# ku222/Attention-GAN

Hardware: AMD Instinct MI355X
Metric: train images/sec at 256×256 stage-3, batch 24/GPU, 1/2/4/8 MI355X (higher is better)
Workload: dtype f32; 1 GPU; full 3-stage AttnGAN 64->128->256 train step: G + 3xD updates + word attention + DAMSM words/sentence loss + KL + 4x fused Adam (BASELINE.json configs[2]); workload_key=full3, batch_per_gpu=24, global_batch=24, gf_dim=32, df_dim=64, emb_dim=256, seq_len=10, text_encoder=bypassed (frozen; N(0,1) embeddings), parallelism=dp1, discriminator_streams=3, launch=eager, gradient_exchange=none (one rank), losses_finite=True

## Files before the change

### attention-gan_amd/csrc/conv.hip

```cpp
#include "conv_common.h"

#include <cxxabi.h>
#include <cstdlib>


using namespace agan;

using namespace agan::conv;

namespace {

__global__ __launch_bounds__(256) void ktable_kernel(int2* __restrict__ tab, int n, int K, int RS, int S, int IHW, int IW, int DY) {
    const int k = blockIdx.x * 256 + threadIdx.x;
    if (k >= n) return;
    int2 a, b;
    if (k < K) {
        const int c = k / RS, rs = k - c * RS, r = rs / S, q = rs - r * S;
        const int dy = r * DY, dx = q * DY;
        a.x = c * IHW + dy * IW + dx;
        a.y = (dy & 0xFFFF) | (dx << 16);
        b.x = c * IHW * 4;
        b.y = rs * kTapRowBytes;
    } else {
        a.x = 0;
// ... 723 lines not shown
                int rl, rh;
                up_fwd_taps(py, r, rl, rh);
                if (a < rl || a > rh) continue;
                for (int px = 0; px < 2; ++px)
                    for (int q = 0; q < 2; ++q) {
                        int sl, sh;
                        up_fwd_taps(px, q, sl, sh);
                        if (b < sl || b > sh) continue;
                        v += dwk[((size_t)(py * 2 + px) * cout + co) * K + (ci * 4 + r * 2 + q)];
                    }
            }
        dw[e] = accumulate ? dw[e] + v : v;
    }
}

__global__ __launch_bounds__(256) void bias_grad_kernel(const float* __restrict__ dy, float* __restrict__ db, int B, int C,
                                                        int HW, int accumulate) {
    __shared__ float red[4];
    const int c = blockIdx.x;
    float s = 0.f;
    for (int b = 0; b < B; ++b) {
        const float* p = dy + ((size_t)b * C + c) * HW;
        for (int i = threadIdx.x; i < HW; i += 256) s += p[i];
    }
    s = block_sum<256>(s, red);
    if (threadIdx.x == 0) db[c] = accumulate ? db[c] + s : s;
}

}

static thread_local hipEvent_t g_timer_start = nullptr, g_timer_stop = nullptr;
static thread_local const void* g_timed_kernel = nullptr;
static thread_local int g_timed_split = 0;
namespace agan { namespace conv { thread_local const void* g_noted_kernel = nullptr; } }
static inline void timer_begin(hipStream_t st) {
    if (g_timer_start) (void)hipEventRecord(g_timer_start, st);
}
static inline void timer_end(hipStream_t st, int split) {
    if (g_timer_stop) {
        (void)hipEventRecord(g_timer_stop, st);
        g_timed_kernel = agan::conv::g_noted_kernel;
        g_timed_split = split;
    }
    g_timer_start = g_timer_stop = nullptr;
}
namespace agan { namespace conv {
void timed_begin(hipStream_t st) { timer_begin(st); }
void timed_end(hipStream_t st, int split) { timer_end(st, split); }
} }

static bool dt16(int dt) { return dt == AGAN_DT_BF16 || dt == AGAN_DT_F16; }
static int mode_dtype(int mode) { return mode == AGAN_PREC_BF16 ? AGAN_DT_BF16 : (mode == AGAN_PREC_F16 ? AGAN_DT_F16 : AGAN_DT_F32); }

enum class GatherPath { none, p16, patch, winograd, small_n, direct };
struct GatherRoute {
    int mode = AGAN_PREC_F32;
    GatherPath path = GatherPath::none;
    P16Plan p16{};
    PatchPlan pp{};
    PatchGather patch{};
    WinoPlan wino{};
    GatherPlan direct{};
    size_t ws_bytes = 0;
    int split = 1;
};

static GatherRoute route_gather(const agan_conv_geom* gg, int prec, int in_dtype, int out_dtype, bool epilogue) {
    GatherRoute r;
    auto take = [&r](GatherPath path, size_t ws_bytes, int split) {
        r.path = path;
        r.ws_bytes = ws_bytes;
        r.split = split;
        return r;
    };
    if (check_geom(gg)) return r;
    const Geom g = make_geom(gg);
    if (prec_planes(prec) > 0 && patch_supported(g)) r.mode = prec;
    const bool f32io = in_dtype == AGAN_DT_F32 && out_dtype == AGAN_DT_F32;
    if (const int want = mode_dtype(r.mode)) {
        if ((in_dtype == AGAN_DT_F32 || in_dtype == want) && (out_dtype == AGAN_DT_F32 || out_dtype == want)) {
            r.p16 = plan_p16(g, in_dtype != AGAN_DT_F32);
            if (r.p16.ok) return take(GatherPath::p16, r.p16.ws_bytes, r.p16.ksplit);
        }
    }
    if (r.mode != AGAN_PREC_F32) {
        if (!f32io) return r;
        r.pp = make_patch_plan(g);
        r.patch = plan_patch_gather(g, r.pp);
        return take(GatherPath::patch, r.patch.ws_bytes, r.patch.ksplit);
    }
    if (f32io && !epilogue) {
        r.wino = plan_wino(g);
        if (r.wino.ok) return take(GatherPath::winograd, r.wino.ws_bytes, r.wino.ksplit);
    }
    if (small_n_gather_supported(g)) {
        const bool linear = g.RS == 1 && g.IH == 1 && g.IW == 1;
        if ((in_dtype == AGAN_DT_F32 || (dt16(in_dtype) && !linear)) && out_dtype == AGAN_DT_F32) return take(GatherPath::small_n, 0, 1);
        return r;
    }
    if (in_dtype == AGAN_DT_F32 && (out_dtype == AGAN_DT_F32 || dt16(out_dtype))) {
        r.direct = plan_gather(g, AGAN_PREC_F32);
        return take(GatherPath::direct, r.direct.ws_bytes, r.direct.ksplit);
    }
    return r;
}

enum class WgradPath { none, winograd, rows, patch, small_n, direct };
struct WgradRoute {
    int mode = AGAN_PREC_F32;
    WgradPath path = WgradPath::none;
    WinoWgradPlan wino{};
    RowsPlan rows{};
    PatchPlan pp{};
    PatchWgrad patch{};
    SmallWgradPlan small{};
    WgradPlan direct{};
    size_t ws_bytes = 0;
    int split = 1;
};

static WgradRoute route_wgrad(const agan_conv_geom* gg, int pack_mode, int prec, int x_dtype, int dy_dtype) {
    WgradRoute r;
    auto take = [&r](WgradPath path, size_t ws_bytes, int split) {
        r.path = path;
        r.ws_bytes = ws_bytes;
        r.split = split;
        return r;
    };
    if (check_geom(gg)) return r;
    const Geom g = make_geom(gg);
    const bool up = pack_mode == AGAN_PACK_UP_FWD, x16 = x_dtype != AGAN_DT_F32, y16 = dy_dtype != AGAN_DT_F32;
    if (prec_planes(prec) > 0 && patch_supported(g)) {
        r.mode = prec;
        if (prec == AGAN_PREC_BF16X6) r.mode = AGAN_PREC_F16X3;
        if (up && !plan_rows_wgrad(g, r.mode, false, false, true).ok) r.mode = AGAN_PREC_F32;
    }
    if (x16 || y16) {
        const int want = mode_dtype(r.mode);
        const bool ok = r.mode == AGAN_PREC_F32
                            ? pack_mode == AGAN_PACK_FWD && small_n_wgrad_supported(g) && dt16(x_dtype) && !y16
                            : want != AGAN_DT_F32 && (!x16 || x_dtype == want) && (!y16 || dy_dtype == want);
        if (!ok) return r;
    }
    if (r.mode == AGAN_PREC_F32 && !up && !x16 && !y16) {
        r.wino = plan_wino_wgrad(g);
        if (r.wino.ok) return take(WgradPath::winograd, r.wino.ws_bytes, r.wino.psplit);
    }
    if (!(r.mode == AGAN_PREC_F32 && small_n_wgrad_supported(g))) {
        r.rows = plan_rows_wgrad(g, r.mode, x16, y16, up);
        if (r.rows.ok) return take(WgradPath::rows, r.rows.ws_bytes, r.rows.psplit);
    }
    if (r.mode != AGAN_PREC_F32) {
        r.pp = make_patch_plan(g);
        r.patch = plan_patch_wgrad(g, r.pp, r.mode);
        return take(WgradPath::patch, r.patch.ws_bytes, r.patch.psplit);
    }
    if (!up && small_n_wgrad_supported(g)) {
        r.small = plan_wgrad_small_n(g);
        return take(WgradPath::small_n, r.small.ws_bytes, r.small.nchunk);
    }
    if (!x16 && !y16) {
        r.direct = plan_wgrad(g, up);
        return take(WgradPath::direct, r.direct.ws_bytes, r.direct.psplit);
    }
    return r;
}

static int check_ws(const char* who, size_t need, const void* ws, size_t ws_bytes) {
    if (need > ws_bytes || (need && !ws)) {
        set_error("%s: workspace %zu < %zu", who, ws_bytes, need);
        return AGAN_EWORKSPACE;
    }
    return AGAN_OK;
}

template <class Launch>
static int launch_main(hipStream_t st, int split, const char* what, Launch&& launch) {
    timer_begin(st);
    launch();
    timer_end(st, split);
    return check_launch(what);
}

extern "C" {

int agan_timer_last_kernel(char* name, size_t capacity) {
    AGAN_REQUIRE(name && capacity > 1, "timer_last_kernel: bad argument");
    name[0] = 0;
    if (!g_timed_kernel) return AGAN_OK;
    const char* mangled = hipKernelNameRefByPtr(g_timed_kernel, nullptr);
    if (!mangled) return AGAN_OK;
    int status = 0;
    char* dem = abi::__cxa_demangle(mangled, nullptr, nullptr, &status);
    const char* src = (status == 0 && dem) ? dem : mangled;
    strncpy(name, src, capacity - 1);
    name[capacity - 1] = 0;
    free(dem);
    return AGAN_OK;
}

int agan_timer_last_split(void) { return g_timed_kernel ? g_timed_split : 0; }

int agan_timer_create(void** event) {
    AGAN_REQUIRE(event != nullptr, "timer_create: null pointer");
    hipEvent_t e;
    if (hipEventCreate(&e) != hipSuccess) {
        set_error("timer_create: hipEventCreate failed");
        return AGAN_ELAUNCH;
    }
    *event = e;
    return AGAN_OK;
}
int agan_timer_destroy(void* event) { return (event && hipEventDestroy(static_cast<hipEvent_t>(event)) != hipSuccess) ? AGAN_ELAUNCH : AGAN_OK; }
// ... 114 lines not shown
    return route_gather(gg, prec, in_dtype, out_dtype, false).path != GatherPath::none ? 1 : 0;
}

int agan_conv_gather_dt(const void* in_v, const void* wkv, const float* bias, void* out_v, const agan_conv_geom* gg, const int32_t* ktable,
                        int prec, int act, const void* lrelu_mask_v, void* ws, size_t ws_bytes, void* stream, const float* in_scale,
                        float* out_amax, int in_dtype, int out_dtype) {
    if (int e = check_geom(gg)) return e;
    AGAN_REQUIRE(in_v && wkv && out_v && ktable, "conv_gather: null pointer");
    AGAN_REQUIRE(act == AGAN_ACT_NONE || (act == AGAN_ACT_LRELU && gg->Cout > 4),
                 "conv_gather: fused activation %d not available for this call (MFMA paths, LeakyReLU only)", act);
    AGAN_REQUIRE(!lrelu_mask_v || (gg->Cout > 4 && act == AGAN_ACT_NONE),
                 "conv_gather: the LeakyReLU-derivative mask needs an MFMA path and no other activation");
    AGAN_REQUIRE(prec == AGAN_PREC_F32 || prec_planes(prec) > 0, "conv_gather: unknown precision mode %d", prec);
    const GatherRoute r = route_gather(gg, prec, in_dtype, out_dtype, bias || act != AGAN_ACT_NONE || lrelu_mask_v);
    AGAN_REQUIRE(r.mode == prec,
                 "conv_gather: precision mode %d does not take this geometry (agan_conv_effective_prec says which one does)", prec);
    AGAN_REQUIRE(r.path != GatherPath::none,
                 "conv_gather: 16-bit activation storage (%d -> %d) is not available for this geometry / precision %d "
                 "(agan_conv_gather_dt_supported)", in_dtype, out_dtype, prec);
    AGAN_REQUIRE(prec != AGAN_PREC_F16X3 || in_scale != nullptr, "conv_gather: AGAN_PREC_F16X3 needs the operand's agan_absmax_scale pair");
    if (int e = check_ws("conv_gather", r.ws_bytes, ws, ws_bytes)) return e;
    const Geom g = make_geom(gg);
    hipStream_t st = as_stream(stream);
    const float* in = static_cast<const float*>(in_v);
    const float* wk = static_cast<const float*>(wkv);
    const float* lrelu_mask = static_cast<const float*>(lrelu_mask_v);
    void* dst = r.split > 1 ? ws : out_v;
    const float* slabs = static_cast<const float*>(ws);
    size_t slab = 0;
    float* sum_amax = nullptr;
    int e = AGAN_OK;
    switch (r.path) {
        case GatherPath::p16:
            slab = r.p16.slab;
            e = launch_main(st, r.split, "conv_gather/p16", [&] {
                launch_p16_gather(in_v, wkv, bias, dst, g, r.p16, prec, act, lrelu_mask_v, st, in_dtype != AGAN_DT_F32, out_dtype != AGAN_DT_F32);
            });
            break;
        case GatherPath::patch:
            slab = r.patch.slab;
            sum_amax = out_amax;
            e = launch_main(st, r.split, "conv_gather/patch", [&] {
                launch_patch_gather(in, wkv, bias, static_cast<float*>(dst), g, r.pp, r.patch, prec, act, lrelu_mask, st, in_scale, out_amax);
            });
            break;
        case GatherPath::winograd:
            slab = r.wino.slab;
            slabs = reinterpret_cast<const float*>(static_cast<const char*>(ws) + r.wino.u_bytes);
            e = launch_main(st, r.split, "conv_gather/winograd", [&] { launch_wino(in, wk, static_cast<float*>(out_v), g, r.wino, ws, st); });
            break;
        case GatherPath::small_n:
            e = launch_main(st, r.split, "conv_gather/small_n", [&] { launch_gather_small_n(in_v, wk, bias, static_cast<float*>(out_v), g, st, in_dtype); });
            break;
        default: {
            const GatherPlan& p = r.direct;
            slab = p.slab;
            const int2* ktab = reinterpret_cast<const int2*>(ktable);
            e = launch_main(st, r.split, "conv_gather", [&] {
                if (p.bn == 128) launch_gather<128, 2, 2>(in, wk, bias, dst, ktab, g, p, act, lrelu_mask_v, st, out_dtype);
                else if (p.bn == 64) launch_gather<64, 2, 2>(in, wk, bias, dst, ktab, g, p, act, lrelu_mask_v, st, out_dtype);
                else launch_gather<32, 4, 1>(in, wk, bias, dst, ktab, g, p, act, lrelu_mask_v, st, out_dtype);
            });
        }
    }
    if (e || r.split == 1) return e;
    launch_sum_slabs(slabs, r.split, (size_t)g.B * g.Cout * g.OH * g.OW, slab, bias, g.Cout, g.OH * g.OW, out_v, 0, act, lrelu_mask_v, sum_amax, st,
                     out_dtype);
    return check_launch("conv_gather/sum_slabs");
}

int agan_conv_gather(const float* in, const void* wkv, const float* bias, float* out, const agan_conv_geom* gg, const int32_t* ktable,
                     int prec, int act, const float* lrelu_mask, void* ws, size_t ws_bytes, void* stream, const float* in_scale,
                     float* out_amax) {
    return agan_conv_gather_dt(in, wkv, bias, out, gg, ktable, prec, act, lrelu_mask, ws, ws_bytes, stream, in_scale, out_amax,
                               AGAN_DT_F32, AGAN_DT_F32);
}

static const int kPrecs[] = {AGAN_PREC_F32, AGAN_PREC_BF16, AGAN_PREC_BF16X3, AGAN_PREC_F16, AGAN_PREC_BF16X6, AGAN_PREC_F16X3};

size_t agan_conv_wgrad_ws_bytes(const agan_conv_geom* g) {
    if (check_geom(g)) return 0;
    const int pack_mode = g->OS == 2 ? AGAN_PACK_UP_FWD : AGAN_PACK_FWD;
    size_t a = 0;
    for (int prec : kPrecs)
        for (int x_dtype : kDtypes)
            for (int dy_dtype : kDtypes) a = std::max(a, route_wgrad(g, pack_mode, prec, x_dtype, dy_dtype).ws_bytes);
    return a;
}

int agan_conv_wgrad_dt_supported(const agan_conv_geom* gg, int pack_mode, int prec, int x_dtype, int dy_dtype) {
    return route_wgrad(gg, pack_mode, prec, x_dtype, dy_dtype).path != WgradPath::none ? 1 : 0;
}

int agan_conv_wgrad(const float* x, const float* dy, float* dw, const agan_conv_geom* gg, const int32_t* ktable, int pack_mode,
                    int kh, int kw, int prec, int accumulate, void* ws, size_t ws_bytes, void* stream, const float* x_scale,
                    const float* dy_scale) {
    return agan_conv_wgrad_dt(x, dy, dw, gg, ktable, pack_mode, kh, kw, prec, accumulate, ws, ws_bytes, stream, x_scale, dy_scale,
                              AGAN_DT_F32, AGAN_DT_F32);
}

int agan_conv_wgrad_dt(const void* x_v, const void* dy_v, float* dw, const agan_conv_geom* gg, const int32_t* ktable, int pack_mode,
                       int kh, int kw, int prec, int accumulate, void* ws, size_t ws_bytes, void* stream, const float* x_scale,
                       const float* dy_scale, int x_dtype, int dy_dtype) {
    const WgradRoute r = route_wgrad(gg, pack_mode, prec, x_dtype, dy_dtype);
    AGAN_REQUIRE(r.path != WgradPath::none,
                 "conv_wgrad: 16-bit activation storage (%d, %d) is not available for this geometry / precision %d", x_dtype, dy_dtype, prec);
    AGAN_REQUIRE(x_v && dy_v && dw && ktable, "conv_wgrad: null pointer");
    AGAN_REQUIRE(prec == AGAN_PREC_F32 || prec_planes(prec) > 0, "conv_wgrad: unknown precision mode %d", prec);
    AGAN_REQUIRE(pack_mode == AGAN_PACK_FWD || pack_mode == AGAN_PACK_UP_FWD, "conv_wgrad: pack mode %d is not a forward mode", pack_mode);
    const Geom g = make_geom(gg);
    const bool up = pack_mode == AGAN_PACK_UP_FWD;
    AGAN_REQUIRE(1LL * g.B * g.Cin * g.IH * g.IW < (1LL << 29) && 1LL * g.B * g.Cout * g.OH * g.OW < (1LL << 29),
                 "conv_wgrad: tensor exceeds 2^29 elements");
    if (!up) AGAN_REQUIRE(g.R == kh && g.S == kw && g.OS == 1, "conv_wgrad: geometry is not a direct %dx%d conv", kh, kw);
    else AGAN_REQUIRE(g.R == 2 && g.S == 2 && g.OS == 2 && kh == 3 && kw == 3, "conv_wgrad: geometry is not the folded upsample conv");
    AGAN_REQUIRE(r.mode != AGAN_PREC_F16X3 || (x_scale && dy_scale),
                 "conv_wgrad: precision mode %d runs this weight gradient as AGAN_PREC_F16X3 (agan_conv_wgrad_effective_prec), which needs the "
                 "amax slots of x and dy (x_amax / dy_amax)", prec);
    if (int e = check_ws("conv_wgrad", r.ws_bytes, ws, ws_bytes)) return e;
    hipStream_t st = as_stream(stream);
    const float* x = static_cast<const float*>(x_v);
    const float* dy = static_cast<const float*>(dy_v);
    float* wsf = static_cast<float*>(ws);
    const bool x16 = x_dtype != AGAN_DT_F32, y16 = dy_dtype != AGAN_DT_F32;
    switch (r.path) {
        case WgradPath::winograd:
            if (int e = launch_main(st, r.split, "conv_wgrad/winograd", [&] { launch_wino_wgrad(x, dy, wsf, g, r.wino, st); })) return e;
            launch_wino_wgrad_sum(wsf, g, r.wino, dw, accumulate ? 1 : 0, st);
            return check_launch("conv_wgrad/winograd/sum");
        case WgradPath::rows:
        case WgradPath::patch: {
            const bool rows = r.path == WgradPath::rows;
            int e;
            if (rows) e = launch_main(st, r.split, "conv_wgrad/rows", [&] {
                launch_rows_wgrad(x_v, dy_v, wsf, g, r.rows, r.mode, st, x_scale, dy_scale, x16, y16);
            });
            else e = launch_main(st, r.split, "conv_wgrad/patch", [&] {
                launch_patch_wgrad(x_v, dy_v, wsf, g, r.pp, r.patch, r.mode, st, x_scale, dy_scale, x16, y16);
            });
            if (e) return e;
            const size_t slab = rows ? r.rows.slab : r.patch.slab;
            const int NPH = rows ? r.rows.NPH : r.pp.NPH, NT = rows ? r.rows.NT : r.pp.NT, Kp = rows ? r.rows.Kp : r.patch.Kp;
            const int ncls = rows ? 1 : r.patch.ncls;
            const bool unfold = up && !rows;
            float* reduced = r.split > 1 ? wsf + slab * r.split : wsf;
            const bool sum_first = unfold ? r.split > 1 : r.split > 4;
            if (sum_first) {
                launch_sum_slabs(wsf, r.split, (size_t)ncls * g.Cout * Kp, slab, nullptr, 1, 1, reduced, 0, AGAN_ACT_NONE, nullptr, nullptr, st);
                if (int e2 = check_launch("conv_wgrad/sum_slabs")) return e2;
            }
            if (unfold) launch_patch_wgrad_unpack(reduced, dw, g.Cout, g.Cin, kh, kw, up, r.pp, r.patch, accumulate, st);
            else launch_wgrad_sum_unpack(sum_first ? reduced : wsf, sum_first ? 1 : r.split, slab, dw, g.Cout, g.Cin, kh, kw, NPH, NT, Kp, accumulate, st);
            return check_launch("conv_wgrad/unpack");
        }
        case WgradPath::small_n: {
            if (int e = launch_main(st, r.split, "conv_wgrad/small_n", [&] { launch_wgrad_small_n(x_v, dy, wsf, g, r.small, st, x_dtype); })) return e;
            launch_sum_slabs(wsf, r.split, (size_t)g.Cout * g.K, r.small.slab, nullptr, 1, 1, dw, accumulate, AGAN_ACT_NONE, nullptr, nullptr, st);
            return check_launch("conv_wgrad/small_n/sum_slabs");
        }
        default: {
            const WgradPlan& p = r.direct;
            const int acc_in_kernel = (accumulate && !up && p.psplit == 1) ? 1 : 0;
            const bool via_sum = p.psplit > 1 || (accumulate && !up && !acc_in_kernel);
            float* reduced = up ? wsf + (p.psplit > 1 ? p.slab * p.psplit : 0) : dw;
            float* part = via_sum ? wsf : reduced;
            const int2* ktab = reinterpret_cast<const int2*>(ktable);
            dim3 grid(p.itiles, p.jtiles, p.ncls * p.psplit);
#define AGAN_WG(BI, BJ) AGAN_LAUNCH((conv_wgrad_f32_kernel<BI, BJ>), grid, dim3(256), 0, st, x, dy, part, ktab, g, p.psplit, p.pchunk, p.slab, acc_in_kernel)
            const int e = launch_main(st, r.split, "conv_wgrad", [&] {
                if (p.bi == 128 && p.bj == 128) AGAN_WG(128, 128);
                else if (p.bi == 128) AGAN_WG(128, 64);
                else if (p.bj == 128) AGAN_WG(64, 128);
                else AGAN_WG(64, 64);
            });
#undef AGAN_WG
            if (e) return e;
            if (via_sum) {
                launch_sum_slabs(part, p.psplit, (size_t)p.ncls * g.Cout * g.K, p.slab, nullptr, 1, 1, reduced, (accumulate && !up) ? 1 : 0,
                                 AGAN_ACT_NONE, nullptr, nullptr, st);
                if (int e2 = check_launch("conv_wgrad/sum_slabs")) return e2;
            }
            if (up) {
                const size_t total = (size_t)g.Cout * g.Cin * 9;
                AGAN_LAUNCH(unpack_wgrad_up_kernel, dim3((unsigned)std::min<size_t>(cdivz(total, 256), 4096)), dim3(256), 0, st,
                            reduced, dw, g.Cout, g.Cin, accumulate);
                return check_launch("conv_wgrad/unpack");
            }
            return AGAN_OK;
        }
    }
}

int agan_bias_grad(const float* dy, float* dbias, int B, int C, int HW, int accumulate, void* stream) {
    AGAN_REQUIRE(dy && dbias && B > 0 && C > 0 && HW > 0, "bias_grad: bad argument");
    AGAN_LAUNCH(bias_grad_kernel, dim3(C), dim3(256), 0, as_stream(stream), dy, dbias, B, C, HW, accumulate);
    return check_launch("bias_grad");
}

static int conv2d_geom(const agan_conv2d_desc* d, int dgrad, Geom& g, int& pack_mode) {
    AGAN_REQUIRE(d != nullptr, "conv2d: null descriptor");
    AGAN_REQUIRE(d->B > 0 && d->Cin > 0 && d->IH > 0 && d->IW > 0 && d->Cout > 0 && d->OH > 0 && d->OW > 0, "conv2d: non-positive dimension");
    AGAN_REQUIRE(d->KH > 0 && d->KW > 0 && d->KH * d->KW <= kMaxTaps2d, "conv2d: %dx%d taps unsupported (at most %d)", d->KH, d->KW, kMaxTaps2d);
    AGAN_REQUIRE((d->SH == 1 || d->SH == 2) && (d->SW == 1 || d->SW == 2), "conv2d: strides %dx%d unsupported (1 or 2 per axis)", d->SH, d->SW);
    AGAN_REQUIRE(d->PH >= 0 && d->PW >= 0 && d->PH < d->KH && d->PW < d->KW, "conv2d: padding %dx%d unsupported for %dx%d taps", d->PH, d->PW,
                 d->KH, d->KW);
    AGAN_REQUIRE(d->OH == (d->IH + 2 * d->PH - d->KH) / d->SH + 1 && d->OW == (d->IW + 2 * d->PW - d->KW) / d->SW + 1 &&
                     d->IH + 2 * d->PH >= d->KH && d->IW + 2 * d->PW >= d->KW,
                 "conv2d: output %dx%d does not match input %dx%d, taps %dx%d, stride %dx%d, padding %dx%d", d->OH, d->OW, d->IH, d->IW, d->KH,
                 d->KW, d->SH, d->SW, d->PH, d->PW);
    AGAN_REQUIRE(d->in_c0 >= 0 && d->in_c0 + d->Cin <= d->in_ctot && d->out_c0 >= 0 && d->out_c0 + d->Cout <= d->out_ctot,
                 "conv2d: channel slice out of range (in %d+%d of %d, out %d+%d of %d)", d->in_c0, d->Cin, d->in_ctot, d->out_c0, d->Cout,
                 d->out_ctot);
// ... 103 lines not shown
```

### attention-gan_amd/csrc/conv_common.h

```cpp
#pragma once
#include "agan_common.h"

#include <algorithm>
#include <type_traits>

namespace agan {
namespace conv {

typedef float f32x16 __attribute__((ext_vector_type(16)));

extern thread_local const void* g_noted_kernel;
#define AGAN_LAUNCH(kernel, ...)                                                   \
    do {                                                                           \
        ::agan::conv::g_noted_kernel = reinterpret_cast<const void*>(kernel);      \
        hipLaunchKernelGGL(kernel, __VA_ARGS__);                                   \
    } while (0)
void timed_begin(hipStream_t st);
void timed_end(hipStream_t st, int split);


struct FastDiv {
    unsigned mul, shift;
    __device__ __forceinline__ int div(int n) const { return (int)((__umulhi(mul, (unsigned)n) + (unsigned)n) >> shift); }
};
// ... 159 lines not shown
    p.ntiles = cdiv(g.Cout, p.bn);
    p.ncls = g.OS * g.OS;
    const int tiles = p.mtiles * p.ntiles * p.ncls;
    const int ktiles = cdiv(g.K, bk);
    int ks = 1;
    if (tiles < slots) ks = std::max(1, std::min({slots / tiles, std::max(1, ktiles / 16), 32}));
    p.kchunk = cdiv(ktiles, ks) * bk;
    p.ksplit = cdiv(g.K, p.kchunk);
    p.slab = (size_t)g.B * g.Cout * g.OH * g.OW;
    p.slab = (p.slab + 3) / 4 * 4;
    p.ws_bytes = p.ksplit > 1 ? p.slab * p.ksplit * sizeof(float) : 0;
    return p;
}

struct WgradPlan {
    int bi, bj, itiles, jtiles, ncls, psplit, pchunk;
    size_t slab, ws_bytes;
};

inline WgradPlan plan_wgrad(const Geom& g, bool needs_combine) {
    WgradPlan p;
    p.bi = (g.K >= 96 && cdiv(g.K, 128) * 128 <= cdiv(g.K, 64) * 64) ? 128 : 64;
    p.bj = g.Cout >= 96 ? 128 : 64;
    p.itiles = cdiv(g.K, p.bi);
    p.jtiles = cdiv(g.Cout, p.bj);
    p.ncls = g.OS * g.OS;
    const int tiles = p.itiles * p.jtiles * p.ncls;
    const int ptiles = cdiv(g.Mtot, 32);
    int ps = 1;
    if (tiles < 512) {
        const int cap = std::max(1, ptiles / 4);
        const int ps1 = std::max(1, std::min(512 / tiles, cap)), ps2 = std::max(1, std::min(1024 / tiles, cap));
        const double fill1 = (double)tiles * ps1 / 512.0, fill2 = (double)tiles * ps2 / 1024.0;
        ps = std::min(fill2 > fill1 + 1e-9 ? ps2 : ps1, 2048);
    }
    p.pchunk = cdiv(ptiles, ps) * 32;
    p.psplit = cdiv(g.Mtot, p.pchunk);
    p.slab = ((size_t)p.ncls * g.Cout * g.K + 3) / 4 * 4;
    const size_t nslabs = p.psplit + (needs_combine ? 1 : 0);
    p.ws_bytes = p.slab * nslabs * sizeof(float);
    return p;
}

struct SmallWgradPlan {
    int pchunk, nchunk;
    size_t slab, ws_bytes;
};
bool small_n_gather_supported(const Geom& g);
void launch_gather_small_n(const void* in, const float* wk, const float* bias, float* out, const Geom& g, hipStream_t st, int in_dtype = AGAN_DT_F32);
bool small_n_wgrad_supported(const Geom& g);
SmallWgradPlan plan_wgrad_small_n(const Geom& g);
void launch_wgrad_small_n(const void* x, const float* dy, float* part, const Geom& g, const SmallWgradPlan& p, hipStream_t st, int x_dtype = AGAN_DT_F32);

__host__ __device__ inline void pack_taps(int mode, int kh, int kw, int& R, int& S, int& SY) {
    switch (mode) {
        case AGAN_PACK_DGRAD_4x4S2: case AGAN_PACK_UP_FWD: R = S = 2; SY = 1; return;
        case AGAN_PACK_UP_DGRAD: R = S = 4; SY = 2; return;
        default: R = kh; S = kw; SY = (kh == 4) ? 2 : 1; return;
    }
}
struct PatchPlan {
    int twl, thl;
    int tiles_x, tiles_y, tiles_b, mtiles;
    int PW, PH, PHW, PP;
    int NPH, NT, IS;
    int nchunks, nstages, nsteps;
    int tapoff[9];
    int tappos[9];
    int base_y[2][2], base_x[2][2];
    FastDiv dPP, dPHW, dPW;
    FastDiv dNT, dNCLS, dMT, dTX, dTY, dNPH, dNPH2;
    int g_ntiles, g_ncls;
};
struct PatchGather {
    int bn, ntiles, ncls, ksplit, stages_per_split;
    size_t slab, ws_bytes;
};
struct PatchWgrad {
    int bj, jtiles, ncls, psplit, tiles_per_split, Kp;
    size_t slab, ws_bytes;
};
struct P16Plan {
    int ok;
    int gk;
    int twl, thl, TB;
    int tiles_x, tiles_y, tiles_b, mtiles;
    int PH, PW, LW, NXB, PXB, CHS;
    int nitems, NI;
    int nstages, wsteps;
    int bn, ntiles, ncls, ksplit, stages_per_split;
    int buf_bytes, smem_bytes;
    int lds_epi;
    int px2;
    int wc, lp;
    size_t slab, ws_bytes;
    FastDiv dNXB, dPH, dTB, dNT, dNCLS, dMT, dTX, dTY;
};
P16Plan plan_p16(const Geom& g, bool in16);
void launch_p16_gather(const void* in, const void* wk, const float* bias, void* dst, const Geom& g, const P16Plan& p, int prec, int act,
                       const void* lrelu_mask, hipStream_t st, bool in16, bool out16);
struct RowsPlan {
    int ok, gk, ci2, ups;
    int twl, thl, tbl;
    int tiles_x, tiles_y, tiles_b, mtiles;
    int XR, XRT;
    int rowb, cpitch;
// ... 63 lines not shown
```

### attention-gan_amd/csrc/conv_small.hip

```cpp
#include "conv_common.h"

using namespace agan;
using namespace agan::conv;

namespace {

template <int RS, int S, int IDT = AGAN_DT_F32>
__global__ __launch_bounds__(256) void conv_small_n_kernel(const void* __restrict__ in, const float* __restrict__ wk,
                                                           const float* __restrict__ bias, float* __restrict__ out, const Geom g) {
    int F = xcd_contiguous(linear_block_id(), (int)(gridDim.x * gridDim.y));
    const int cls = F % (int)gridDim.y;
    F /= (int)gridDim.y;
    const int py = cls / g.OS, px = cls - py * g.OS;
    const int m = F * 256 + threadIdx.x;
    const bool valid = m < g.Mtot;
    const int mm = valid ? m : 0;
    const int b = g.dHWs.div(mm), rem = mm - b * g.HWs;
    const int yq = g.dOWs.div(rem), xq = rem - yq * g.OWs;
    const int iy0 = yq * g.SY + (py ? g.OY1 : g.OY0), ix0 = xq * g.SY + (px ? g.OY1 : g.OY0);
    const int ihw = g.IH * g.IW;
    const int pix0 = b * g.Cin * ihw + iy0 * g.IW + ix0;
    unsigned off[RS];
#pragma unroll
    for (int t = 0; t < RS; ++t) {
// ... 252 lines not shown
                        const int row = py - r + 1, col = px - t + 1;
#pragma unroll
                        for (int p = 0; p < 4; ++p)
#pragma unroll
                            for (int n = 0; n < NC; ++n) acc[k][p][n] += w[n] * v[row][p + col];
                    }
            }
        }
    }
    if (CS > 1) {
        __shared__ float red[CS - 1 > 0 ? CS - 1 : 1][16 * NC][64];
        const int lane = threadIdx.x & 63;
        __syncthreads();
        if (wave > 0) {
#pragma unroll
            for (int k = 0; k < 4; ++k)
#pragma unroll
                for (int p = 0; p < 4; ++p)
#pragma unroll
                    for (int n = 0; n < NC; ++n) red[wave - 1][(k * 4 + p) * NC + n][lane] = acc[k][p][n];
        }
        __syncthreads();
        if (wave > 0) return;
#pragma unroll
        for (int w = 0; w < CS - 1; ++w)
#pragma unroll
            for (int k = 0; k < 4; ++k)
#pragma unroll
                for (int p = 0; p < 4; ++p)
#pragma unroll
                    for (int n = 0; n < NC; ++n) acc[k][p][n] += red[w][(k * 4 + p) * NC + n][lane];
    }
    if (!valid) return;
#pragma unroll
    for (int n = 0; n < NC; ++n) {
        if (n >= g.Cout) break;
        const float bv = bias ? bias[n] : 0.f;
#pragma unroll
        for (int py = 0; py < 2; ++py) {
            float q[8];
#pragma unroll
            for (int p = 0; p < 4; ++p)
#pragma unroll
                for (int px = 0; px < 2; ++px)
                    q[2 * p + px] = acc[py * 2 + px][p][n] + bv;
            float* o = out + (((size_t)b * g.Cout + n) * g.OH + (2 * y + py)) * g.OW + xs * 8;
            *reinterpret_cast<float4*>(o) = make_float4(q[0], q[1], q[2], q[3]);
            *reinterpret_cast<float4*>(o + 4) = make_float4(q[4], q[5], q[6], q[7]);
        }
    }
}

__global__ __launch_bounds__(256) void linear_small_n_kernel(const float* __restrict__ in, const float* __restrict__ wk,
                                                             const float* __restrict__ bias, float* __restrict__ out, int K, int Nld, int Cout) {
    __shared__ float red[4][4];
    const int m = blockIdx.x;
    const float* x = in + (size_t)m * K;
    float a[4] = {0.f, 0.f, 0.f, 0.f};
    for (int k = threadIdx.x; k < K; k += 256) {
        const float v = x[k];
        const float4 w = *reinterpret_cast<const float4*>(wk + (size_t)k * Nld);
        a[0] += v * w.x; a[1] += v * w.y; a[2] += v * w.z; a[3] += v * w.w;
    }
#pragma unroll
    for (int n = 0; n < 4; ++n) a[n] = wave_sum(a[n]);
    const int w = threadIdx.x >> 6;
    if ((threadIdx.x & 63) == 0)
        for (int n = 0; n < 4; ++n) red[n][w] = a[n];
    __syncthreads();
    if (threadIdx.x < Cout) {
        const int n = threadIdx.x;
        out[(size_t)m * Cout + n] = red[n][0] + red[n][1] + red[n][2] + red[n][3] + (bias ? bias[n] : 0.f);
    }
}

template <int RS, int S, int XDT = AGAN_DT_F32>
__global__ __launch_bounds__(256) void wgrad_small_n_kernel(const void* __restrict__ x, const float* __restrict__ dy, float* __restrict__ part,
                                                            const Geom g, const int pchunk, const size_t slab) {
    __shared__ float red[4][RS * 4];
    const int F = xcd_contiguous(linear_block_id(), (int)(gridDim.x * gridDim.y));
    const int c = F % (int)gridDim.x, chunk = F / (int)gridDim.x;
    const int pbeg = chunk * pchunk, pend = min(g.Mtot, pbeg + pchunk);
    const int ihw = g.IH * g.IW, ohw = g.OH * g.OW;
    constexpr unsigned XE = XDT == AGAN_DT_F32 ? 4u : 2u;
    const __amdgpu_buffer_rsrc_t rx = make_rsrc(x, (size_t)g.B * g.Cin * ihw * XE);
    const unsigned soff = (unsigned)(c * ihw) * XE;
    float acc[RS][4];
#pragma unroll
    for (int t = 0; t < RS; ++t)
#pragma unroll
        for (int n = 0; n < 4; ++n) acc[t][n] = 0.f;
    for (int p = pbeg + threadIdx.x; p < pend; p += 256) {
        const int b = g.dHWs.div(p), rem = p - b * g.HWs;
        const int yq = g.dOWs.div(rem), xq = rem - yq * g.OWs;
        const int iy0 = yq * g.SY + g.OY0, ix0 = xq * g.SY + g.OY0;
        const int pix0 = b * g.Cin * ihw + iy0 * g.IW + ix0;
        const float* dp = dy + (size_t)b * g.Cout * ohw + (size_t)yq * g.OW + xq;
        float d[4];
#pragma unroll
        for (int n = 0; n < 4; ++n) d[n] = n < g.Cout ? dp[(size_t)n * ohw] : 0.f;
#pragma unroll
        for (int t = 0; t < RS; ++t) {
            const int ddy = (t / S) * g.DY, ddx = (t % S) * g.DY;
            const bool ok = ((unsigned)(iy0 + ddy) < (unsigned)g.IH) & ((unsigned)(ix0 + ddx) < (unsigned)g.IW);
            float v;
            if (XDT == AGAN_DT_F32) v = buf_load_s(rx, ok ? (unsigned)(pix0 + ddy * g.IW + ddx) * 4u : kOOB, soff);
            else {
                const unsigned short h = (unsigned short)__builtin_amdgcn_raw_buffer_load_b16(rx, ok ? (unsigned)(pix0 + ddy * g.IW + ddx) * 2u : kOOB, soff, 0);
                v = XDT == AGAN_DT_BF16 ? __uint_as_float((unsigned)h << 16) : (float)__builtin_bit_cast(_Float16, h);
            }
#pragma unroll
            for (int n = 0; n < 4; ++n) acc[t][n] += v * d[n];
        }
    }
    const int w = threadIdx.x >> 6, lane = threadIdx.x & 63;
// ... 59 lines not shown
                    const float xv = v[r][p + t];
#pragma unroll
                    for (int n = 0; n < NC; ++n) acc[r * 3 + t][n] += P.dyr[n][p] * xv;
                }
    };
    Pass A, B;
    if (sbeg < send) issue(sbeg, A);
    for (int s0 = sbeg; s0 < send; s0 += 512) {
        const bool more1 = s0 + 256 < send, more2 = s0 + 512 < send;
        if (more1) issue(s0 + 256, B);
        consume(A);
        if (more1) {
            if (more2) issue(s0 + 512, A);
            consume(B);
        }
    }
    const int w = threadIdx.x >> 6, lane = threadIdx.x & 63;
#pragma unroll
    for (int t = 0; t < 9; ++t)
#pragma unroll
        for (int n = 0; n < NC; ++n) {
            const float sum = wave_sum(acc[t][n]);
            if (lane == 0) red[w][t * 4 + n] = sum;
        }
    __syncthreads();
    if (threadIdx.x < 36) {
        const int t = threadIdx.x >> 2, n = threadIdx.x & 3;
        if (n < NC && n < g.Cout)
            part[(size_t)chunk * slab + (size_t)n * g.K + c * 9 + t] =
                red[0][threadIdx.x] + red[1][threadIdx.x] + red[2][threadIdx.x] + red[3][threadIdx.x];
    }
}

bool strip_ok(const Geom& g) {
    return g.RS == 9 && g.S == 3 && g.OS == 1 && g.SY == 1 && g.DY == 1 && g.OY0 == -1 && g.IH == g.OH && g.IW == g.OW && (g.IW & 3) == 0 && g.Cout <= 4;
}
bool dgrad4_strip_ok(const Geom& g) {
    return g.R == 2 && g.S == 2 && g.OS == 2 && g.SY == 1 && g.DY == -1 && g.OY0 == 0 && g.OY1 == 1 && g.OH == 2 * g.IH && g.OW == 2 * g.IW &&
           (g.IW & 3) == 0 && g.Cout <= 4;
}

}

namespace agan {
namespace conv {

bool small_n_gather_supported(const Geom& g) {
    if (g.Cout > 4 || g.R != g.S) return false;
    return g.RS == 1 || g.RS == 4 || g.RS == 9 || g.RS == 16;
}

void launch_gather_small_n(const void* in, const float* wk, const float* bias, float* out, const Geom& g, hipStream_t st, int in_dtype) {
    if (g.RS == 1 && g.IH == 1 && g.IW == 1 && g.OS == 1 && g.SY == 1 && g.OY0 == 0) {
        AGAN_LAUNCH(linear_small_n_kernel, dim3(g.Mtot), dim3(256), 0, st, static_cast<const float*>(in), wk, bias, out, g.K, g.Nld, g.Cout);
        return;
    }
    if (strip_ok(g)) {
        const int nstrips = g.B * g.IH * (g.IW >> 2);
        const bool split = nstrips <= 64 * 1024 && g.Cin >= 8;
        const dim3 sg(split ? cdiv(nstrips, 64) : cdiv(nstrips, 256));
#define AGAN_STRIP2(NC_, CS_)                                                                                                             \
    do {                                                                                                                                  \
        if (in_dtype == AGAN_DT_BF16) AGAN_LAUNCH((conv_small_strip_kernel<AGAN_DT_BF16, NC_, CS_>), sg, dim3(256), 0, st, in, wk, bias, out, g); \
        else if (in_dtype == AGAN_DT_F16) AGAN_LAUNCH((conv_small_strip_kernel<AGAN_DT_F16, NC_, CS_>), sg, dim3(256), 0, st, in, wk, bias, out, g); \
        else AGAN_LAUNCH((conv_small_strip_kernel<AGAN_DT_F32, NC_, CS_>), sg, dim3(256), 0, st, in, wk, bias, out, g);                  \
    } while (0)
#define AGAN_STRIP(NC_) do { if (split) AGAN_STRIP2(NC_, 4); else AGAN_STRIP2(NC_, 1); } while (0)
        if (g.Cout <= 2) AGAN_STRIP(2);
        else if (g.Cout == 3) AGAN_STRIP(3);
        else AGAN_STRIP(4);
#undef AGAN_STRIP
#undef AGAN_STRIP2
        return;
    }
    if (dgrad4_strip_ok(g)) {
        const int nstrips = g.B * g.IH * (g.IW >> 2);
        const bool split = nstrips <= 64 * 1024 && g.Cin >= 8;
        const dim3 sg(split ? cdiv(nstrips, 64) : cdiv(nstrips, 256));
#define AGAN_STRIP2(NC_, CS_)                                                                                                             \
    do {                                                                                                                                  \
        if (in_dtype == AGAN_DT_BF16) AGAN_LAUNCH((conv_small_dgrad4_strip_kernel<AGAN_DT_BF16, NC_, CS_>), sg, dim3(256), 0, st, in, wk, bias, out, g); \
        else if (in_dtype == AGAN_DT_F16) AGAN_LAUNCH((conv_small_dgrad4_strip_kernel<AGAN_DT_F16, NC_, CS_>), sg, dim3(256), 0, st, in, wk, bias, out, g); \
        else AGAN_LAUNCH((conv_small_dgrad4_strip_kernel<AGAN_DT_F32, NC_, CS_>), sg, dim3(256), 0, st, in, wk, bias, out, g);           \
    } while (0)
#define AGAN_STRIP(NC_) do { if (split) AGAN_STRIP2(NC_, 4); else AGAN_STRIP2(NC_, 1); } while (0)
        if (g.Cout <= 2) AGAN_STRIP(2);
        else if (g.Cout == 3) AGAN_STRIP(3);
        else AGAN_STRIP(4);
#undef AGAN_STRIP
#undef AGAN_STRIP2
        return;
    }
    dim3 grid(cdiv(g.Mtot, 256), g.OS * g.OS);
#define AGAN_SN(RS_, S_)                                                                                                                  \
    do {                                                                                                                                  \
        if (in_dtype == AGAN_DT_BF16) AGAN_LAUNCH((conv_small_n_kernel<RS_, S_, AGAN_DT_BF16>), grid, dim3(256), 0, st, in, wk, bias, out, g); \
        else if (in_dtype == AGAN_DT_F16) AGAN_LAUNCH((conv_small_n_kernel<RS_, S_, AGAN_DT_F16>), grid, dim3(256), 0, st, in, wk, bias, out, g); \
        else AGAN_LAUNCH((conv_small_n_kernel<RS_, S_>), grid, dim3(256), 0, st, in, wk, bias, out, g);                              \
    } while (0)
    switch (g.RS) {
        case 1: AGAN_SN(1, 1); break;
        case 4: AGAN_SN(4, 2); break;
        case 9: AGAN_SN(9, 3); break;
        default: AGAN_SN(16, 4); break;
    }
#undef AGAN_SN
}
// ... 36 lines not shown
```

Baseline: 998.6 images/s.

## Add dedicated streaming kernels for linear (1x1 on 1x1) forward and weight-gradient

Adds a linear-geometry route for small batches (B<=64): a weight-streaming GEMV-like kernel that stages activations in LDS, splits K across blocks and reduces across waves, plus a dedicated weight-gradient kernel. It also vectorizes and unrolls the existing small-N linear kernel with float4 loads. The goal is to replace the generic gather/wgrad paths for the FC layers (fc 200->16384, CA-net, D logits), which are memory-bound on weight reads. The cost is new code paths and split-K slab reductions for small layers.

```diff
diff --git a/attention-gan_amd/csrc/conv.hip b/attention-gan_amd/csrc/conv.hip
--- a/attention-gan_amd/csrc/conv.hip
+++ b/attention-gan_amd/csrc/conv.hip
@@ -799,7 +799,7 @@
 static bool dt16(int dt) { return dt == AGAN_DT_BF16 || dt == AGAN_DT_F16; }
 static int mode_dtype(int mode) { return mode == AGAN_PREC_BF16 ? AGAN_DT_BF16 : (mode == AGAN_PREC_F16 ? AGAN_DT_F16 : AGAN_DT_F32); }
 
-enum class GatherPath { none, p16, patch, winograd, small_n, direct };
+enum class GatherPath { none, p16, patch, winograd, small_n, linear, direct };
 struct GatherRoute {
     int mode = AGAN_PREC_F32;
     GatherPath path = GatherPath::none;
@@ -807,6 +807,7 @@
     PatchPlan pp{};
     PatchGather patch{};
     WinoPlan wino{};
+    LinearPlan linear{};
     GatherPlan direct{};
     size_t ws_bytes = 0;
     int split = 1;
@@ -845,6 +846,10 @@
         if ((in_dtype == AGAN_DT_F32 || (dt16(in_dtype) && !linear)) && out_dtype == AGAN_DT_F32) return take(GatherPath::small_n, 0, 1);
         return r;
     }
+    if (f32io && linear_geometry(g)) {
+        r.linear = plan_linear(g);
+        return take(GatherPath::linear, r.linear.ws_bytes, r.linear.ksplit);
+    }
     if (in_dtype == AGAN_DT_F32 && (out_dtype == AGAN_DT_F32 || dt16(out_dtype))) {
         r.direct = plan_gather(g, AGAN_PREC_F32);
         return take(GatherPath::direct, r.direct.ws_bytes, r.direct.ksplit);
@@ -852,7 +857,7 @@
     return r;
 }
 
-enum class WgradPath { none, winograd, rows, patch, small_n, direct };
+enum class WgradPath { none, winograd, rows, patch, small_n, linear, direct };
 struct WgradRoute {
     int mode = AGAN_PREC_F32;
     WgradPath path = WgradPath::none;
@@ -906,6 +911,7 @@
         r.small = plan_wgrad_small_n(g);
         return take(WgradPath::small_n, r.small.ws_bytes, r.small.nchunk);
     }
+    if (!up && !x16 && !y16 && linear_geometry(g)) return take(WgradPath::linear, 0, 1);
     if (!x16 && !y16) {
         r.direct = plan_wgrad(g, up);
         return take(WgradPath::direct, r.direct.ws_bytes, r.direct.psplit);
@@ -1126,6 +1132,12 @@
         case GatherPath::small_n:
             e = launch_main(st, r.split, "conv_gather/small_n", [&] { launch_gather_small_n(in_v, wk, bias, static_cast<float*>(out_v), g, st, in_dtype); });
             break;
+        case GatherPath::linear:
+            slab = r.linear.slab;
+            e = launch_main(st, r.split, "conv_gather/linear", [&] {
+                launch_linear(in, wk, bias, static_cast<float*>(dst), g, r.linear, act, lrelu_mask, st);
+            });
+            break;
         default: {
             const GatherPlan& p = r.direct;
             slab = p.slab;
@@ -1232,6 +1244,8 @@
             launch_sum_slabs(wsf, r.split, (size_t)g.Cout * g.K, r.small.slab, nullptr, 1, 1, dw, accumulate, AGAN_ACT_NONE, nullptr, nullptr, st);
             return check_launch("conv_wgrad/small_n/sum_slabs");
         }
+        case WgradPath::linear:
+            return launch_main(st, r.split, "conv_wgrad/linear", [&] { launch_linear_wgrad(x, dy, dw, g, accumulate ? 1 : 0, st); });
         default: {
             const WgradPlan& p = r.direct;
             const int acc_in_kernel = (accumulate && !up && p.psplit == 1) ? 1 : 0;
diff --git a/attention-gan_amd/csrc/conv_common.h b/attention-gan_amd/csrc/conv_common.h
--- a/attention-gan_amd/csrc/conv_common.h
+++ b/attention-gan_amd/csrc/conv_common.h
@@ -235,6 +235,18 @@
 SmallWgradPlan plan_wgrad_small_n(const Geom& g);
 void launch_wgrad_small_n(const void* x, const float* dy, float* part, const Geom& g, const SmallWgradPlan& p, hipStream_t st, int x_dtype = AGAN_DT_F32);
 
+constexpr int kLinearRows = 64;
+struct LinearPlan {
+    int mr, mgroups, ntiles;
+    int ksplit, kchunk;
+    size_t slab, ws_bytes;
+};
+bool linear_geometry(const Geom& g);
+LinearPlan plan_linear(const Geom& g);
+void launch_linear(const float* x, const float* wk, const float* bias, float* dst, const Geom& g, const LinearPlan& p, int act,
+                   const float* lrelu_mask, hipStream_t st);
+void launch_linear_wgrad(const float* x, const float* dy, float* dw, const Geom& g, int accumulate, hipStream_t st);
+
 __host__ __device__ inline void pack_taps(int mode, int kh, int kw, int& R, int& S, int& SY) {
     switch (mode) {
         case AGAN_PACK_DGRAD_4x4S2: case AGAN_PACK_UP_FWD: R = S = 2; SY = 1; return;
diff --git a/attention-gan_amd/csrc/conv_small.hip b/attention-gan_amd/csrc/conv_small.hip
--- a/attention-gan_amd/csrc/conv_small.hip
+++ b/attention-gan_amd/csrc/conv_small.hip
@@ -328,15 +328,39 @@
 }
 
 __global__ __launch_bounds__(256) void linear_small_n_kernel(const float* __restrict__ in, const float* __restrict__ wk,
-                                                             const float* __restrict__ bias, float* __restrict__ out, int K, int Nld, int Cout) {
+                                                             const float* __restrict__ bias, float* __restrict__ out, int K, int Nld, int Cout,
+                                                             int vec) {
     __shared__ float red[4][4];
     const int m = blockIdx.x;
     const float* x = in + (size_t)m * K;
     float a[4] = {0.f, 0.f, 0.f, 0.f};
-    for (int k = threadIdx.x; k < K; k += 256) {
-        const float v = x[k];
-        const float4 w = *reinterpret_cast<const float4*>(wk + (size_t)k * Nld);
-        a[0] += v * w.x; a[1] += v * w.y; a[2] += v * w.z; a[3] += v * w.w;
+    if (vec) {
+        constexpr int U = 4;
+        const int K4 = K >> 2;
+        for (int q0 = threadIdx.x; q0 < K4; q0 += 256 * U) {
+            f32x4 xv[U], wv[U][4];
+#pragma unroll
+            for (int u = 0; u < U; ++u) {
+                const int q = q0 + 256 * u;
+                const bool ok = q < K4;
+                xv[u] = ok ? *reinterpret_cast<const f32x4*>(x + (size_t)q * 4) : f32x4{0.f, 0.f, 0.f, 0.f};
+#pragma unroll
+                for (int j = 0; j < 4; ++j)
+                    wv[u][j] = ok ? *reinterpret_cast<const f32x4*>(wk + ((size_t)q * 4 + j) * Nld) : f32x4{0.f, 0.f, 0.f, 0.f};
+            }
+#pragma unroll
+            for (int u = 0; u < U; ++u)
+#pragma unroll
+                for (int j = 0; j < 4; ++j)
+#pragma unroll
+                    for (int n = 0; n < 4; ++n) a[n] += xv[u][j] * wv[u][j][n];
+        }
+    } else {
+        for (int k = threadIdx.x; k < K; k += 256) {
+            const float v = x[k];
+            const float4 w = *reinterpret_cast<const float4*>(wk + (size_t)k * Nld);
+            a[0] += v * w.x; a[1] += v * w.y; a[2] += v * w.z; a[3] += v * w.w;
+        }
     }
 #pragma unroll
     for (int n = 0; n < 4; ++n) a[n] = wave_sum(a[n]);
@@ -502,7 +526,8 @@
 
 void launch_gather_small_n(const void* in, const float* wk, const float* bias, float* out, const Geom& g, hipStream_t st, int in_dtype) {
     if (g.RS == 1 && g.IH == 1 && g.IW == 1 && g.OS == 1 && g.SY == 1 && g.OY0 == 0) {
-        AGAN_LAUNCH(linear_small_n_kernel, dim3(g.Mtot), dim3(256), 0, st, static_cast<const float*>(in), wk, bias, out, g.K, g.Nld, g.Cout);
+        const int vec = (g.K & 3) == 0 && (reinterpret_cast<uintptr_t>(in) & 15) == 0 ? 1 : 0;
+        AGAN_LAUNCH(linear_small_n_kernel, dim3(g.Mtot), dim3(256), 0, st, static_cast<const float*>(in), wk, bias, out, g.K, g.Nld, g.Cout, vec);
         return;
     }
     if (strip_ok(g)) {
diff --git a/attention-gan_amd/csrc/linear.hip b/attention-gan_amd/csrc/linear.hip
--- /dev/null
+++ b/attention-gan_amd/csrc/linear.hip
@@ -0,0 +1,212 @@
+#include "conv_common.h"
+
+using namespace agan;
+using namespace agan::conv;
+
+namespace {
+
+constexpr int kLinKC = 128;
+constexpr int kLinU = 8;
+
+template <int MR>
+__global__ __launch_bounds__(256) void linear_stream_kernel(const float* __restrict__ x, const float* __restrict__ wk, const float* __restrict__ bias,
+                                                            float* __restrict__ dst, const float* __restrict__ lrelu_mask, int M, int K, int N, int Nld,
+                                                            int kchunk, size_t slab, int lrelu, int vec) {
+    __shared__ __attribute__((aligned(16))) float xs[kLinKC * MR];
+    __shared__ __attribute__((aligned(16))) float red[3][32][64];
+    const int tid = threadIdx.x, lane = tid & 63;
+    const int w = __builtin_amdgcn_readfirstlane(tid >> 6);
+    const int m0 = blockIdx.z * MR, rows = min(MR, M - m0);
+    const int kbeg = blockIdx.y * kchunk, kend = min(K, kbeg + kchunk);
+    const int n0 = blockIdx.x * 256 + lane * 4;
+    const bool live = n0 < Nld;
+    float acc[MR][4];
+#pragma unroll
+    for (int m = 0; m < MR; ++m)
+#pragma unroll
+        for (int c = 0; c < 4; ++c) acc[m][c] = 0.f;
+    for (int k0 = kbeg; k0 < kend; k0 += kLinKC) {
+        const int kc = min(kLinKC, kend - k0);
+        __syncthreads();
+        for (int idx = tid; idx < kc * MR; idx += 256) {
+            const int m = idx % MR, kk = idx / MR;
+            xs[idx] = m < rows ? x[(size_t)(m0 + m) * K + (k0 + kk)] : 0.f;
+        }
+        __syncthreads();
+        for (int kk0 = w; kk0 < kc; kk0 += 4 * kLinU) {
+            f32x4 wv[kLinU];
+#pragma unroll
+            for (int u = 0; u < kLinU; ++u) {
+                const int kk = kk0 + 4 * u;
+                wv[u] = f32x4{0.f, 0.f, 0.f, 0.f};
+                if (live && kk < kc) wv[u] = *reinterpret_cast<const f32x4*>(wk + (size_t)(k0 + kk) * Nld + n0);
+            }
+#pragma unroll
+            for (int u = 0; u < kLinU; ++u) {
+                const int kk = kk0 + 4 * u;
+                if (kk < kc) {
+#pragma unroll
+                    for (int m4 = 0; m4 < MR / 4; ++m4) {
+                        const f32x4 xv = *reinterpret_cast<const f32x4*>(&xs[kk * MR + m4 * 4]);
+#pragma unroll
+                        for (int j = 0; j < 4; ++j)
+#pragma unroll
+                            for (int c = 0; c < 4; ++c) acc[m4 * 4 + j][c] += xv[j] * wv[u][c];
+                    }
+                }
+            }
+        }
+    }
+#pragma unroll
+    for (int r0 = 0; r0 < MR; r0 += 8) {
+        __syncthreads();
+        if (w > 0) {
+#pragma unroll
+            for (int r = 0; r < 8; ++r)
+#pragma unroll
+                for (int c = 0; c < 4; ++c) red[w - 1][r * 4 + c][lane] = acc[r0 + r][c];
+        }
+        __syncthreads();
+        if (w == 0) {
+#pragma unroll
+            for (int s = 0; s < 3; ++s)
+#pragma unroll
+                for (int r = 0; r < 8; ++r)
+#pragma unroll
+                    for (int c = 0; c < 4; ++c) acc[r0 + r][c] += red[s][r * 4 + c][lane];
+        }
+    }
+    if (w > 0 || n0 >= N) return;
+    const bool split = gridDim.y > 1;
+    float* out = split ? dst + (size_t)blockIdx.y * slab : dst;
+#pragma unroll
+    for (int m = 0; m < MR; ++m) {
+        if (m >= rows) continue;
+        const size_t o = (size_t)(m0 + m) * N + n0;
+        float v[4];
+#pragma unroll
+        for (int c = 0; c < 4; ++c) {
+            v[c] = acc[m][c];
+            if (!split) {
+                const bool in = n0 + c < N;
+                if (bias && in) v[c] += bias[n0 + c];
+                if (lrelu) v[c] = v[c] > 0.f ? v[c] : 0.2f * v[c];
+                if (lrelu_mask && in) v[c] = lrelu_mask[o + c] > 0.f ? v[c] : 0.2f * v[c];
+            }
+        }
+        if (vec) *reinterpret_cast<f32x4*>(out + o) = f32x4{v[0], v[1], v[2], v[3]};
+        else {
+#pragma unroll
+            for (int c = 0; c < 4; ++c)
+                if (n0 + c < N) out[o + c] = v[c];
+        }
+    }
+}
+
+template <int P>
+__global__ __launch_bounds__(256) void linear_wgrad_kernel(const float* __restrict__ x, const float* __restrict__ dy, float* __restrict__ dw, int M,
+                                                           int Cin, int Cout, int accumulate, int vec) {
+    constexpr int MRW = 32;
+    __shared__ __attribute__((aligned(16))) float xs[MRW][256];
+    __shared__ __attribute__((aligned(16))) float ds[MRW][4 * P];
+    const int tid = threadIdx.x, q = tid & 63;
+    const int c = __builtin_amdgcn_readfirstlane(tid >> 6);
+    const int co0 = blockIdx.x * 4 * P, ci0 = blockIdx.y * 256;
+    float acc[P][4];
+#pragma unroll
+    for (int p = 0; p < P; ++p)
+#pragma unroll
+        for (int j = 0; j < 4; ++j) acc[p][j] = 0.f;
+    for (int mb = 0; mb < M; mb += MRW) {
+        const int rows = min(MRW, M - mb);
+        __syncthreads();
+        for (int idx = tid; idx < rows * 256; idx += 256) {
+            const int m = idx >> 8, i = idx & 255;
+            xs[m][i] = ci0 + i < Cin ? x[(size_t)(mb + m) * Cin + ci0 + i] : 0.f;
+        }
+        for (int idx = tid; idx < rows * 4 * P; idx += 256) {
+            const int m = idx / (4 * P), j = idx % (4 * P);
+            ds[m][j] = co0 + j < Cout ? dy[(size_t)(mb + m) * Cout + co0 + j] : 0.f;
+        }
+        __syncthreads();
+        for (int m = 0; m < rows; ++m) {
+            const f32x4 xv = *reinterpret_cast<const f32x4*>(&xs[m][q * 4]);
+#pragma unroll
+            for (int p = 0; p < P; ++p) {
+                const float d = ds[m][c * P + p];
+#pragma unroll
+                for (int j = 0; j < 4; ++j) acc[p][j] += d * xv[j];
+            }
+        }
+    }
+    const int ci = ci0 + q * 4;
+    if (ci >= Cin) return;
+#pragma unroll
+    for (int p = 0; p < P; ++p) {
+        const int co = co0 + c * P + p;
+        if (co >= Cout) continue;
+        float* o = dw + (size_t)co * Cin + ci;
+        if (vec) {
+            f32x4 v = {acc[p][0], acc[p][1], acc[p][2], acc[p][3]};
+            if (accumulate) {
+                const f32x4 old = *reinterpret_cast<const f32x4*>(o);
+                v = f32x4{old[0] + v[0], old[1] + v[1], old[2] + v[2], old[3] + v[3]};
+            }
+            *reinterpret_cast<f32x4*>(o) = v;
+        } else {
+#pragma unroll
+            for (int j = 0; j < 4; ++j)
+                if (ci + j < Cin) o[j] = accumulate ? o[j] + acc[p][j] : acc[p][j];
+        }
+    }
+}
+
+bool aligned16(const void* p) { return (reinterpret_cast<uintptr_t>(p) & 15) == 0; }
+
+}
+
+namespace agan {
+namespace conv {
+
+bool linear_geometry(const Geom& g) {
+    return g.IH == 1 && g.IW == 1 && g.OH == 1 && g.OW == 1 && g.R == 1 && g.S == 1 && g.OS == 1 && g.SY == 1 && g.OY0 == 0 && g.B <= kLinearRows;
+}
+
+LinearPlan plan_linear(const Geom& g) {
+    LinearPlan p;
+    p.mr = g.B <= 8 ? 8 : (g.B <= 16 ? 16 : 32);
+    p.mgroups = cdiv(g.B, p.mr);
+    p.ntiles = cdiv(g.Nld, 256);
+    const int blocks = p.ntiles * p.mgroups;
+    const int ks = std::max(1, std::min(256 / blocks, g.K / 32));
+    p.kchunk = cdiv(g.K, ks);
+    p.ksplit = cdiv(g.K, p.kchunk);
+    p.slab = ((size_t)g.B * g.Cout + 3) / 4 * 4;
+    p.ws_bytes = p.ksplit > 1 ? p.slab * p.ksplit * sizeof(float) : 0;
+    return p;
+}
+
+void launch_linear(const float* x, const float* wk, const float* bias, float* dst, const Geom& g, const LinearPlan& p, int act,
+                   const float* lrelu_mask, hipStream_t st) {
+    const dim3 grid(p.ntiles, p.ksplit, p.mgroups);
+    const int vec = (g.Cout & 3) == 0 && aligned16(dst) ? 1 : 0;
+    const int lrelu = act == AGAN_ACT_LRELU ? 1 : 0;
+#define AGAN_LIN(MR_) AGAN_LAUNCH((linear_stream_kernel<MR_>), grid, dim3(256), 0, st, x, wk, bias, dst, lrelu_mask, g.B, g.K, g.Cout, g.Nld, p.kchunk, p.slab, lrelu, vec)
+    if (p.mr == 8) AGAN_LIN(8);
+    else if (p.mr == 16) AGAN_LIN(16);
+    else AGAN_LIN(32);
+#undef AGAN_LIN
+}
+
+void launch_linear_wgrad(const float* x, const float* dy, float* dw, const Geom& g, int accumulate, hipStream_t st) {
+    const int citiles = cdiv(g.Cin, 256);
+    const int P = cdiv(g.Cout, 64) * citiles >= 256 ? 16 : (cdiv(g.Cout, 16) * citiles >= 256 ? 4 : 1);
+    const dim3 grid(cdiv(g.Cout, 4 * P), citiles);
+    const int vec = (g.Cin & 3) == 0 && aligned16(dw) ? 1 : 0;
+    if (P == 16) AGAN_LAUNCH((linear_wgrad_kernel<16>), grid, dim3(256), 0, st, x, dy, dw, g.B, g.Cin, g.Cout, accumulate, vec);
+    else if (P == 4) AGAN_LAUNCH((linear_wgrad_kernel<4>), grid, dim3(256), 0, st, x, dy, dw, g.B, g.Cin, g.Cout, accumulate, vec);
+    else AGAN_LAUNCH((linear_wgrad_kernel<1>), grid, dim3(256), 0, st, x, dy, dw, g.B, g.Cin, g.Cout, accumulate, vec);
+}
+
+}
+}
diff --git a/profiles/linear_micro.py b/profiles/linear_micro.py
--- /dev/null
+++ b/profiles/linear_micro.py
@@ -0,0 +1,110 @@
+#!/usr/bin/env python3
+import ctypes
+import importlib
+import os
+import statistics
+import sys
+from ctypes import byref
+
+import torch
+
+ROOT = os.path.dirname(os.path.dirname(os.path.abspath(__file__)))
+sys.path.insert(0, ROOT)
+HF = importlib.import_module("attention-gan_amd.backend.functional")
+L = HF.L
+
+WINDOW, ROUNDS, WARM = 50, 15, 3
+ROWS = [
+    ("fc 200 -> 16384", "fwd", 24, 200, 16384, 1), ("fc 200 -> 16384", "dgrad", 24, 200, 16384, 1), ("fc 200 -> 16384", "wgrad", 24, 200, 16384, 1),
+    ("CA-net 256 -> 400", "fwd", 24, 256, 400, 1), ("CA-net 256 -> 400", "wgrad", 24, 256, 400, 1),
+    ("D logits 8192 -> 1", "fwd", 48, 8192, 1, 3), ("D logits 8192 -> 1", "fwd", 24, 8192, 1, 3),
+    ("D logits 8192 -> 1", "dgrad", 48, 8192, 1, 3), ("D logits 8192 -> 1", "dgrad", 24, 8192, 1, 3),
+    ("D logits 8192 -> 1", "wgrad", 48, 8192, 1, 3),
+]
+
+
+def make_call(phase, B, K, N, dev):
+    gf, pf, gd, pd, _ = HF.conv_geoms("same", B, K, 1, 1, N, 1)
+    x = torch.randn(B, K, 1, 1, device=dev)
+    w = torch.randn(N, K, 1, 1, device=dev) * 0.05
+    dy = torch.randn(B, N, 1, 1, device=dev)
+    lib = L.load()
+    if phase == "wgrad":
+        dw = torch.empty_like(w)
+        nbytes = lib.agan_conv_wgrad_ws_bytes(byref(gf))
+        ws, wsp = HF._ws(nbytes, x)
+        kt = HF.ktable(gf, dev)
+
+        def call():
+            L.call("agan_conv_wgrad_dt", HF._p(x), HF._p(dy), HF._p(dw), byref(gf), HF._p(kt), pf, 1, 1, L.PREC_F32, 0, wsp, nbytes,
+                   HF._stream(), None, None, L.DT_F32, L.DT_F32)
+        call.keep = (x, dy, dw, ws, kt)
+        return call, 4 * (B * K + B * N + N * K)
+    g, mode, src = (gf, pf, x) if phase == "fwd" else (gd, pd, dy)
+    out = torch.empty((B, N if phase == "fwd" else K, 1, 1), device=dev)
+    wk = HF.packed_weight(w, mode, None, L.PREC_F32)
+    bias = torch.randn(N, device=dev) if phase == "fwd" else None
+    nbytes = lib.agan_conv_gather_ws_bytes(byref(g), L.PREC_F32)
+    ws, wsp = HF._ws(nbytes, x)
+    kt = HF.ktable(g, dev)
+
+    def call():
+        L.call("agan_conv_gather_dt", HF._p(src), HF._p(wk), HF._p(bias), HF._p(out), byref(g), HF._p(kt), L.PREC_F32, 0, None, wsp, nbytes,
+               HF._stream(), None, None, L.DT_F32, L.DT_F32)
+    call.keep = (src, wk, bias, out, ws, kt)
+    return call, 4 * (B * K + B * N + N * K)
+
+
+def main_kernel(call):
+    e0, e1 = ctypes.c_void_p(), ctypes.c_void_p()
+    L.call("agan_timer_create", byref(e0))
+    L.call("agan_timer_create", byref(e1))
+    L.call("agan_timer_arm", e0, e1)
+    call()
+    torch.cuda.synchronize()
+    name = ctypes.create_string_buffer(1024)
+    L.call("agan_timer_last_kernel", name, 1024)
+    split = int(L.load().agan_timer_last_split())
+    L.call("agan_timer_destroy", e0)
+    L.call("agan_timer_destroy", e1)
+    import re
+    m = re.search(r"(\w+_kernel\d*)(<[^()]*>)?", name.value.decode())
+    return ((m.group(1) + (m.group(2) or "")) if m else "?") + (f" /{split}" if split > 1 else "")
+
+
+def main():
+    if not torch.cuda.is_available():
+        sys.exit("linear_micro: needs an MI355X (timings on a CPU say nothing about it)")
+    dev = torch.device("cuda", 0)
+    print(f"library: {os.path.relpath(L.LIB_PATH, ROOT)}; windows of {WINDOW} graph-captured back-to-back calls, median [range] of {ROUNDS} replays")
+    print(f"{'layer':20s} {'phase':6s} {'B':>3s} {'x/step':>6s} {'us/call':>9s} {'range':>17s} {'GB/s':>8s} {'us/step':>8s}  main kernel")
+    total = 0.0
+    for layer, phase, B, K, N, per_step in ROWS:
+        call, owed = make_call(phase, B, K, N, dev)
+        kernel = main_kernel(call)
+        side = torch.cuda.Stream()
+        with torch.cuda.stream(side):
+            for _ in range(3):
+                call()
+            torch.cuda.synchronize()
+            graph = torch.cuda.CUDAGraph()
+            with torch.cuda.graph(graph, stream=side):
+                for _ in range(WINDOW):
+                    call()
+        us = []
+        for r in range(WARM + ROUNDS):
+            e0, e1 = torch.cuda.Event(enable_timing=True), torch.cuda.Event(enable_timing=True)
+            e0.record()
+            graph.replay()
+            e1.record()
+            e1.synchronize()
+            if r >= WARM:
+                us.append(e0.elapsed_time(e1) * 1e3 / WINDOW)
+        med = statistics.median(us)
+        total += med * per_step
+        print(f"{layer:20s} {phase:6s} {B:3d} {per_step:6d} {med:9.2f} [{min(us):7.2f} ..{max(us):7.2f}] {owed / med / 1e3:8.1f} {med * per_step:8.1f}  {kernel}")
+    print(f"sum over the step's {sum(r[5] for r in ROWS)} linear-geometry launches: {total:.1f} us")
+
+
+if __name__ == "__main__":
+    main()
```

New measurement: 998.3 images/s (median of 2 runs). About the same (-0.0%).
